# david8862/tf-keras-speech-commands

Hardware: AMD Instinct MI355X
Metric: 1 s@16 kHz clips/sec train-step, simple_cnn bs4096, 1/2/4/8 MI355X; eval top-1 (higher is better)
Workload: dtype f32; 1 GPU; configs[1]: simple_cnn train step = featurize(f32 1 s @16 kHz) + fwd + bwd + Adam, 36 logits (background + 35 words), batch 4096 per GPU; global_batch=4096, parallelism=dp1, gradient_exchange=none (one rank), rccl_ranks=0, library_build=bf45ad6cdf97

## Files before the change

### tf-keras-speech-commands_amd/csrc/kws_conv.h

```cpp
#pragma once
#include "kws_device.h"

namespace kws {

struct ConvGeom {
    int B, H, W, Ho, Wo;
    int stride, pt, pl;
    int KH, KW;
    int pmajor = 0;
};

enum { EPI_NONE = 0, EPI_RELU = 1, EPI_BIAS_RELU6 = 2, EPI_BIAS = 3, EPI_BIAS_RELU = 4,
       EPI_BN_RELU6 = 5,
       EPI_BNBWD_GATE6 = 6 };
enum { MODE_FWD = 0, MODE_DGRAD = 1 };

__host__ __device__ constexpr int stride16(int c) { return (c % 32 == 16) ? c : c + 16; }

template <int CR, int CO, int MODE, int EPI>
__global__ __launch_bounds__(256) void conv_gemm_kernel(const float *__restrict__ src, const float *__restrict__ wgt,
                                                         const float *__restrict__ bias, float *__restrict__ dst,
                                                         ConvGeom g)
{
    constexpr int KC = CR >= 32 ? 32 : CR;
// ... 1374 lines not shown
template <bool GBN = false>
__global__ __launch_bounds__(256, 2) void conv_wgrad_clip_bf16_kernel(const float *__restrict__ x, const float *__restrict__ dz,
                                                                       float *__restrict__ dw, int B, int H, int W, BnBwdArgs bn)
{
    constexpr int CIN = 16, COUT = 32, KS = 5;
    extern __shared__ __attribute__((aligned(16))) unsigned char ctile[];
    const int lane = threadIdx.x & 63, wave = __builtin_amdgcn_readfirstlane(threadIdx.x >> 6), li = lane & 15, lq = lane >> 4;
    const int nt = wave & 1, tg = wave >> 1;
    const int HP = H + 2, WP = W + 2, HW = H * W, NPIX = HP * WP;
    const int XPL = NPIX * 32, DPL = (HW + 1) * 32;
    unsigned char *Xs = ctile, *Ds = ctile + 3 * XPL;
    for (int i = threadIdx.x; i < (3 * XPL + 6 * DPL) / 4; i += 256) reinterpret_cast<unsigned *>(ctile)[i] = 0u;

    int xaddr[KS][2], daddr[KS][2];
#pragma unroll
    for (int ks = 0; ks < KS; ++ks)
#pragma unroll
        for (int rd = 0; rd < 2; ++rd) {
            const int pq = 32 * ks + 16 * rd + 4 * lq + (li >> 2);
            const bool ok = pq < HW;
            const int oh = ok ? pq / W : 0, ow = ok ? pq - oh * W : 0;
            xaddr[ks][rd] = (oh * WP + ow) * 32 + (li & 3) * 8;
            daddr[ks][rd] = (ok ? pq : HW) * 32 + (li & 3) * 8 + nt * DPL;
        }
    auto frag = [&](const unsigned char *p0, const unsigned char *p1) -> bf16x8 {
        union { struct { s16x4 lo, hi; } s; bf16x8 v; } u;
        u.s.lo = lds_read_tr16(p0);
        u.s.hi = lds_read_tr16(p1);
        return u.v;
    };

    f32x4 acc[5];
#pragma unroll
    for (int t = 0; t < 5; ++t) acc[t] = (f32x4){0.f, 0.f, 0.f, 0.f};

    constexpr int PX = 3, PD = 5;
    const int nx4 = HW * (CIN / 4), nd4 = HW * (COUT / 4);
    f32x4 px[PX], pd[PD], pz[GBN ? PD : 1];
    unsigned pa[GBN ? PD : 1];
    constexpr int F4 = COUT / 4;
    float gi[4], mean[4], inv[4], k2[4], k3[4];
    const int Wp = W / 2, nwin = (H / 2) * Wp;
    int cq[GBN ? PD : 1], ce[GBN ? PD : 1];
    if (GBN) {
#pragma unroll
        for (int e = 0; e < 4; ++e) {
            const int c = 4 * (threadIdx.x % F4) + e;
            inv[e] = bn.inv[c]; gi[e] = bn.gamma[c] * inv[e]; mean[e] = bn.mean[c];
            if (!bn.acc) { k2[e] = bn.k2[c]; k3[e] = bn.k3[c]; }
        }
        if (bn.acc) bn_bwd_k_from_acc(bn, COUT, threadIdx.x % F4, false, k2, k3);
#pragma unroll
        for (int j = 0; j < PD; ++j) {
            const int i = threadIdx.x + 256 * j, pix = i / F4, c4 = i % F4, y = pix / W, xx = pix - y * W;
            const bool in = i < nd4 && y < 2 * (H / 2) && xx < 2 * Wp;
            cq[j] = in ? ((y >> 1) * Wp + (xx >> 1)) * F4 + c4 : -1;
            ce[j] = (y & 1) * 2 + (xx & 1);
        }
    }
    auto prefetch = [&](int b) {
        const f32x4 *xs = reinterpret_cast<const f32x4 *>(x + (long)b * HW * CIN);
#pragma unroll
        for (int j = 0; j < PX; ++j) { const int i = threadIdx.x + 256 * j; px[j] = i < nx4 ? xs[i] : (f32x4){0.f, 0.f, 0.f, 0.f}; }
        if (GBN) {
            const f32x4 *zs = reinterpret_cast<const f32x4 *>(bn.z + (long)b * HW * COUT);
            const f32x4 *gws = reinterpret_cast<const f32x4 *>(bn.gw) + (long)b * nwin * F4;
            const unsigned *ars = reinterpret_cast<const unsigned *>(bn.arg) + (long)b * nwin * F4;
#pragma unroll
            for (int j = 0; j < PD; ++j) {
                const int i = threadIdx.x + 256 * j, q = cq[j] >= 0 ? cq[j] : 0;
                pd[j] = gws[q];
                pa[j] = ars[q];
                pz[j] = i < nd4 ? zs[i] : (f32x4){0.f, 0.f, 0.f, 0.f};
            }
        } else {
            const f32x4 *ds = reinterpret_cast<const f32x4 *>(dz + (long)b * HW * COUT);
#pragma unroll
            for (int j = 0; j < PD; ++j) { const int i = threadIdx.x + 256 * j; pd[j] = i < nd4 ? ds[i] : (f32x4){0.f, 0.f, 0.f, 0.f}; }
        }
    };
    auto form_dz = [&](int j) {
        f32x4 v = pd[j];
#pragma unroll
        for (int e = 0; e < 4; ++e) {
            const float g = (cq[j] >= 0 && (int)((pa[j] >> (8 * e)) & 0xFFu) == ce[j]) ? v[e] : 0.f;
            v[e] = gi[e] * (g - k2[e] - (pz[j][e] - mean[e]) * inv[e] * k3[e]);
        }
        return v;
    };
    auto stage_x = [&](int i, f32x4 v) {
        const int pix = i >> 2, c4 = i & 3, y = pix / W, xx = pix - y * W;
        bf16x4 h, m, l;
        split_bf16(v, h, m, l);
        unsigned char *d = Xs + ((y + 1) * WP + xx + 1) * 32 + c4 * 8;
        *reinterpret_cast<bf16x4 *>(d) = h;
        *reinterpret_cast<bf16x4 *>(d + XPL) = m;
        *reinterpret_cast<bf16x4 *>(d + 2 * XPL) = l;
    };
    auto stage_d = [&](int i, f32x4 v) {
        const int pix = i >> 3, c4 = i & 7;
        bf16x4 h, m, l;
        split_bf16(v, h, m, l);
        unsigned char *d = Ds + (c4 >> 2) * DPL + pix * 32 + (c4 & 3) * 8;
        *reinterpret_cast<bf16x4 *>(d) = h;
        *reinterpret_cast<bf16x4 *>(d + 2 * DPL) = m;
        *reinterpret_cast<bf16x4 *>(d + 4 * DPL) = l;
    };
    if ((int)blockIdx.x < B) prefetch(blockIdx.x);
    for (int b = blockIdx.x; b < B; b += gridDim.x) {
        __syncthreads();
#pragma unroll
        for (int j = 0; j < PX; ++j) { const int i = threadIdx.x + 256 * j; if (i < nx4) stage_x(i, px[j]); }
#pragma unroll
        for (int j = 0; j < PD; ++j) { const int i = threadIdx.x + 256 * j; if (i < nd4) stage_d(i, GBN ? form_dz(j) : pd[j]); }
        if (!GBN && (nx4 > 256 * PX || nd4 > 256 * PD)) {
            const f32x4 *xs = reinterpret_cast<const f32x4 *>(x + (long)b * HW * CIN);
            for (int i = threadIdx.x + 256 * PX; i < nx4; i += 256) stage_x(i, xs[i]);
            const f32x4 *ds = reinterpret_cast<const f32x4 *>(dz + (long)b * HW * COUT);
            for (int i = threadIdx.x + 256 * PD; i < nd4; i += 256) stage_d(i, ds[i]);
        }
        __syncthreads();
        if (b + (int)gridDim.x < B) prefetch(b + gridDim.x);
#pragma unroll
        for (int ks = 0; ks < KS; ++ks) {
            bf16x8 bfr[3];
#pragma unroll
            for (int p = 0; p < 3; ++p) bfr[p] = frag(Ds + 2 * p * DPL + daddr[ks][0], Ds + 2 * p * DPL + daddr[ks][1]);
#pragma unroll
            for (int t = 0; t < 5; ++t) {
                const int tap = tg + 2 * t;
                if (tap < 9) {
                    const int toff = ((tap / 3) * WP + tap % 3) * 32;
                    bf16x8 afr[3];
#pragma unroll
                    for (int p = 0; p < 3; ++p) afr[p] = frag(Xs + p * XPL + toff + xaddr[ks][0], Xs + p * XPL + toff + xaddr[ks][1]);
                    acc[t] = mfma_bf16x6(afr, bfr, acc[t]);
                }
            }
        }
    }
    __syncthreads();
    float *red = reinterpret_cast<float *>(ctile);
#pragma unroll
    for (int t = 0; t < 5; ++t) {
        const int tap = tg + 2 * t;
        if (tap < 9)
#pragma unroll
            for (int r = 0; r < 4; ++r) red[(tap * CIN + 4 * lq + r) * COUT + 16 * nt + li] = acc[t][r];
    }
    __syncthreads();
    for (int idx = threadIdx.x; idx < 9 * CIN * COUT; idx += 256) atomicAdd(dw + idx, red[idx]);
}

template <int COUT>
__global__ __launch_bounds__(256) void conv_wgrad_clip_kernel(const float *__restrict__ x, const float *__restrict__ dz,
                                                               float *__restrict__ dw, int B, int H, int W)
{
    constexpr int CIN = 16, NT = COUT / 16, XS = 16, DS = stride16(COUT);
    extern __shared__ __attribute__((aligned(16))) float smem[];
    const int lane = threadIdx.x & 63, wave = threadIdx.x >> 6, li = lane & 15, lq = lane >> 4;
    const int HP = H + 2, WP = W + 2, HW = H * W, nstep = (HW + 3) / 4;
    float *xt = smem;
    float *dt = smem + HP * WP * XS;
    for (int i = threadIdx.x; i < HP * WP * XS + 4 * nstep * DS; i += 256) smem[i] = 0.f;

    f32x4 acc[9][NT];
#pragma unroll
    for (int t = 0; t < 9; ++t)
#pragma unroll
        for (int nt = 0; nt < NT; ++nt) acc[t][nt] = (f32x4){0.f, 0.f, 0.f, 0.f};

    constexpr int PX = 3, PD = 5;
    const int nx4 = HW * (CIN / 4), nd4 = HW * (COUT / 4);
    float4 px[PX], pd[PD];
    auto prefetch = [&](int b) {
        const float4 *xs = reinterpret_cast<const float4 *>(x + (long)b * HW * CIN);
        const float4 *ds = reinterpret_cast<const float4 *>(dz + (long)b * HW * COUT);
#pragma unroll
        for (int j = 0; j < PX; ++j) { const int i = threadIdx.x + 256 * j; px[j] = i < nx4 ? xs[i] : make_float4(0.f, 0.f, 0.f, 0.f); }
#pragma unroll
        for (int j = 0; j < PD; ++j) { const int i = threadIdx.x + 256 * j; pd[j] = i < nd4 ? ds[i] : make_float4(0.f, 0.f, 0.f, 0.f); }
    };
    if ((int)blockIdx.x < B) prefetch(blockIdx.x);
    for (int b = blockIdx.x; b < B; b += gridDim.x) {
        __syncthreads();
#pragma unroll
        for (int j = 0; j < PX; ++j) {
            const int i = threadIdx.x + 256 * j;
            if (i < nx4) {
                const int pix = i / (CIN / 4), c4 = i % (CIN / 4), y = pix / W, xx = pix % W;
                *reinterpret_cast<float4 *>(&xt[((y + 1) * WP + xx + 1) * XS + 4 * c4]) = px[j];
            }
        }
#pragma unroll
        for (int j = 0; j < PD; ++j) {
            const int i = threadIdx.x + 256 * j;
            if (i < nd4) *reinterpret_cast<float4 *>(&dt[(i / (COUT / 4)) * DS + 4 * (i % (COUT / 4))]) = pd[j];
        }
        if (nx4 > 256 * PX || nd4 > 256 * PD) {
            const float4 *xs = reinterpret_cast<const float4 *>(x + (long)b * HW * CIN);
            for (int i = threadIdx.x + 256 * PX; i < nx4; i += 256) {
                const int pix = i / (CIN / 4), c4 = i % (CIN / 4), y = pix / W, xx = pix % W;
                *reinterpret_cast<float4 *>(&xt[((y + 1) * WP + xx + 1) * XS + 4 * c4]) = xs[i];
            }
            const float4 *ds = reinterpret_cast<const float4 *>(dz + (long)b * HW * COUT);
            for (int i = threadIdx.x + 256 * PD; i < nd4; i += 256)
                *reinterpret_cast<float4 *>(&dt[(i / (COUT / 4)) * DS + 4 * (i % (COUT / 4))]) = ds[i];
        }
        __syncthreads();
        if (b + (int)gridDim.x < B) prefetch(b + gridDim.x);
        for (int st = wave; st < nstep; st += 4) {
            const int p = 4 * st + lq, pc = p < HW ? p : HW - 1;
            const int oh = pc / W, ow = pc % W;
            float bf[NT];
#pragma unroll
            for (int nt = 0; nt < NT; ++nt) bf[nt] = dt[p * DS + 16 * nt + li];
            const float *a0 = &xt[(oh * WP + ow) * XS + li];
#pragma unroll
            for (int kh = 0; kh < 3; ++kh)
#pragma unroll
                for (int kw = 0; kw < 3; ++kw) {
                    const float a = a0[(kh * WP + kw) * XS];
#pragma unroll
                    for (int nt = 0; nt < NT; ++nt) acc[kh * 3 + kw][nt] = mfma16(a, bf[nt], acc[kh * 3 + kw][nt]);
                }
        }
    }
    float *red = smem;
#pragma unroll
    for (int t = 0; t < 9; ++t) {
#pragma unroll
        for (int nt = 0; nt < NT; ++nt) {
            __syncthreads();
            *reinterpret_cast<f32x4 *>(&red[(wave * 64 + lane) * 4]) = acc[t][nt];
            __syncthreads();
            if (wave == 0) {
                const f32x4 s0 = *reinterpret_cast<const f32x4 *>(&red[(0 * 64 + lane) * 4]);
                const f32x4 s1 = *reinterpret_cast<const f32x4 *>(&red[(1 * 64 + lane) * 4]);
                const f32x4 s2 = *reinterpret_cast<const f32x4 *>(&red[(2 * 64 + lane) * 4]);
                const f32x4 s3 = *reinterpret_cast<const f32x4 *>(&red[(3 * 64 + lane) * 4]);
#pragma unroll
                for (int r = 0; r < 4; ++r) red[1024 + (4 * lq + r) * COUT + 16 * nt + li] = (s0[r] + s1[r]) + (s2[r] + s3[r]);
            }
        }
        __syncthreads();
        for (int idx = threadIdx.x; idx < 16 * COUT; idx += 256) atomicAdd(dw + (long)t * CIN * COUT + idx, red[1024 + idx]);
    }
}

}
```

### tf-keras-speech-commands_amd/csrc/kws_model.hip

```cpp
#include <cstdlib>
#include <cstring>
#include <string>
#include <vector>

#include "kws_common.h"
#include "kws_model_types.h"
#include "kws_conv.h"
#include "kws_layers.h"
#include "kws_layer1.h"
#include "kws_layer1_moments.h"
#include "kws_layer1_fast.h"
#include "kws_lite.h"
#include "kws_lite_f16.h"
#include "kws_infer_fused.h"
#include "kws_conv_group.h"
#include "kws_dense_head.h"

using namespace kws;

namespace {

inline int same_out(int n, int s) { return (n + s - 1) / s; }
inline int same_pad_before(int n, int k, int s)
{
// ... 690 lines not shown
        } else if (fused_head) {
            const kws_train_args *a = fused_head;
            const HeadFwdArgs hf{params + m->o_hb, a->labels, a->class_weights, a->probs, w.loss_i, w.correct_i, a->grad_scale / (float)B, a->ignore_index};
            KWS_TRY(run_head_bwd(m, B, params, w.d1, nullptr, w.dd1, grads, true, s, grads + m->o_db, nullptr, nullptr, nullptr, false, &hf));
        } else
            KWS_TRY(run_head_bwd(m, B, params, w.d1, w.dlogits, w.dd1, grads, true, s, fuse && !det ? grads + m->o_db : nullptr, w.loss_i, w.correct_i,
                                 fuse ? stats : nullptr, det));
        fork0_bound = stop_event_bound(fork0_ev);
        if (fused_head) {
            if (fused_head->forward_event) KWS_HIP_CHECK(hipEventRecord(static_cast<hipEvent_t>(fused_head->forward_event), s));
            if (hook) KWS_TRY(hook->fire(1, s));
        }
    }
    {
        ConvGeom g;
        g.B = B; g.H = d.H4; g.W = d.W4; g.Ho = 1; g.Wo = 1; g.stride = 1; g.pt = 0; g.pl = 0; g.KH = d.H4; g.KW = d.W4;
        const bool hook_ev_here = hook && hook->wants(2) && hook->ev;
        if (hook) KWS_TRY(hook->fire(2, s, fork0_bound && hook_ev_here));
        if (hook_ev_here) {
            KWS_HIP_CHECK(hipStreamWaitEvent(s2, fork0_ev, 0));
        } else {
            if (!fork0_bound) KWS_HIP_CHECK(hipEventRecord(R->ev[0], s));
            KWS_HIP_CHECK(hipStreamWaitEvent(s2, R->ev[0], 0));
        }
        if (fused_head && stats) KWS_LAUNCH("loss_reduce_kernel", loss_reduce_kernel, dim3(1), dim3(256), 0, s2, w.loss_i, w.correct_i, B, stats);
        KWS_TRY(launch_wgrad<128, 128, 1>(w.a[3], w.dd1, grads + m->o_dk, g, s2, det));
        int nblk, rows;
        stat_grid(B, 128, nblk, rows);
        if (!head_bwd_fuses(m) || det) {
            KWS_LAUNCH("channel_stats_kernel.dense", channel_stats_kernel, dim3(nblk), dim3(256), 0, s, w.dd1, (long)B, 128, rows, w.partial);
            KWS_LAUNCH("colsum_finalize_kernel", colsum_finalize_kernel, dim3(128), dim3(256), 0, s, w.partial, nblk, 128, grads + m->o_db);
        }
        if (dense_fused) ;
        else if (mprec == 1) KWS_TRY_NB(launch_bf16<128, 128, MODE_DGRAD, EPI_NONE>("conv_bf16_dgrad", w.dd1, w.wsp[2], nullptr, w.da4, g, s));
        else KWS_TRY(launch_dgrad<128, 128, 1>(w.dd1, params + m->o_dk, w.da4, g, s));
        if (hook) KWS_TRY(hook->fire(3, s));
    }
    int fused_bn3_blocks = 0;
    for (int l = 3; l >= 1; --l) {
        if (hook && l == 2) KWS_TRY(hook->fire(5, s));
        const int C = kCh[l + 1];
        const long M = (long)B * Hz[l] * Wz[l];
        const float *da = l == 3 ? w.da4 : w.da[l];
        BnCoef k = coef_of(w.coef[l], C);
        int nblk, rows;
        stat_grid(M, C, nblk, rows);
        const float rate = (l == 3 && seed != 0) ? 0.5f : 0.f;
        const bool compact_g = l == 1 && cnn_compact_g2(m, mprec == 1);
        if (pool[l]) {
            const long NW = (long)B * (Hz[l] / 2) * (Wz[l] / 2);
            stat_grid(NW, C, nblk, rows);
            if (l == 1 && acc_bn2) ;
            else if (l == 3 && acc_bn4) ;
            else if (compact_g && routed_bwd2)
                KWS_LAUNCH(prof_name("bn_bwd_reduce_pool_kernel", l + 1), bn_bwd_reduce_routed_kernel, dim3(nblk), dim3(256), 0, s, w.zmax2, w.da[1], k, NW, C,
                           rows, w.partial);
            else if (compact_g)
                KWS_LAUNCH(prof_name("bn_bwd_reduce_pool_kernel", l + 1), bn_bwd_reduce_pool_kernel<true>, dim3(nblk), dim3(256), 0, s, w.z[l], w.da[1], k,
                           w.gz[l], B, Hz[l], Wz[l], C, rows, w.partial, rate, slo, shi, reinterpret_cast<unsigned char *>(w.da[2]));
            else if (l == 3 && mprec == 1)
                KWS_LAUNCH(prof_name("bn_bwd_reduce_pool_kernel", l + 1), bn_bwd_reduce_routed_full_kernel, dim3(nblk), dim3(256), 0, s, w.zmax4, w.arg4, da, k,
                           w.gz[l], B, Hz[l], Wz[l], C, rows, w.partial, rate, slo, shi);
            else
                KWS_LAUNCH(prof_name("bn_bwd_reduce_pool_kernel", l + 1), bn_bwd_reduce_pool_kernel<false>, dim3(nblk), dim3(256), 0, s, w.z[l],
                           const_cast<float *>(da), k, w.gz[l], B, Hz[l], Wz[l], C, rows, w.partial, rate, slo, shi);
        } else if (l == 2 && fused_bn3_blocks > 0)
            nblk = fused_bn3_blocks;
        else
            KWS_LAUNCH(prof_name("bn_bwd_reduce_kernel", l + 1), bn_bwd_reduce_kernel<false>, dim3(nblk), dim3(256), 0, s, w.z[l], da, k, w.gz[l], B, Hz[l], Wz[l], C,
                       rows, w.partial, rate, slo, shi);
        const bool wgrad_early_l1 = compact_g && Hs[1] * Ws[1] <= 160 && Hs[1] * Ws[1] * 8 <= 1280 && Hs[1] * Ws[1] * 4 <= 768;
        const bool acc_l = (l == 1 && acc_bn2) || (l == 2 && acc_bn3 && fused_bn3_blocks > 0) || (l == 3 && acc_bn4);
        const BnAccBwd ab{acc_set(R, 1, l, bpar[l]), acc_set(R, 1, l, bpar[l] + 1), M, grads + m->o_g[l], grads + m->o_b[l]};
        if (acc_l) ;
        else {
            if (l == 1 && wgrad_early_l1) arm(1);
            KWS_LAUNCH(prof_name("bn_bwd_finalize_kernel", l + 1), bn_bwd_finalize_kernel, dim3(C), dim3(64), 0, s, w.partial, nblk, M, C, params + m->o_g[l],
                       grads + m->o_g[l], grads + m->o_b[l], k);
        }
        if (l != 1) arm(l);
        if (l == 1)
            ;
        else if (l == 3 && acc_bn4)
            KWS_LAUNCH(prof_name("bn_bwd_apply_planes_kernel", l + 1), bn_bwd_apply_routed_planes_kernel<true>, dim3(std::min<unsigned>(1024u, blocks_for(M * C / 4, 256))),
                       dim3(256), 0, s, w.z[l], w.da4, w.arg4, k, params + m->o_g[l], B, Hz[l], Wz[l], C, ab, (Bf16PlanesOut{{w.dzp[0], w.dzp[1], w.dzp[2]}}));
        else if (l == 2 && acc_l)
            KWS_LAUNCH(prof_name("bn_bwd_apply_kernel", l + 1), bn_bwd_apply_acc_kernel<false>, dim3(std::min<unsigned>(1024u, blocks_for(M * C / 4, 256))), dim3(256), 0, s,
                       w.z[l], w.gz[l], k, params + m->o_g[l], M * C / 4, C, ab);
        else if (l == 3 && mprec == 1)
            KWS_LAUNCH(prof_name("bn_bwd_apply_planes_kernel", l + 1), bn_bwd_apply_planes_kernel<true>, dim3(blocks_for(M * C / 4, 256)), dim3(256), 0, s,
                       w.z[l], w.gz[l], k, params + m->o_g[l], M * C / 4, C, (Bf16PlanesOut{{w.dzp[0], w.dzp[1], w.dzp[2]}}));
        else if (l == 3)
            KWS_LAUNCH(prof_name("bn_bwd_apply_kernel", l + 1), bn_bwd_apply_kernel<true>, dim3(blocks_for(M * C, 256)), dim3(256), 0, s, w.z[l], w.gz[l], k,
                       params + m->o_g[l], M * C, C);
        else
            KWS_LAUNCH(prof_name("bn_bwd_apply_kernel", l + 1), bn_bwd_apply_kernel<false>, dim3(blocks_for(M * C, 256)), dim3(256), 0, s, w.z[l], w.gz[l], k,
                       params + m->o_g[l], M * C, C);
        const float *in = w.a[l - 1];
        float *dk = grads + m->o_k[l];
        const float *kern = params + m->o_k[l];
        if (hook && l == 3) KWS_TRY(hook->fire(4, s));
        if (l != 1)
            if (int rc = fork(l)) return rc;
        if (l == 3) {
            const ConvGeom g = geom3x3(B, Hs[3], Ws[3], 1);
            if (mprec == 1 && cnn_a3_on_load(m, true, true))
                KWS_TRY((launch_wgrad_bf16<64, 128, 1, true, true>(w.z[2], nullptr, dk, g, s2, w.dzp, det, coef_of(w.coef[2], 64).scale)));
            else if (mprec == 1) KWS_TRY(launch_wgrad_bf16<64, 128, 1, true>(in, nullptr, dk, g, s2, w.dzp, det));
            else KWS_TRY(launch_wgrad<64, 128, 1>(in, w.gz[3], dk, g, s2, det));
            if (comm) KWS_TRY(comm_allreduce_early(comm, grads + m->o_k[3], m->P - m->o_k[3], s2));
            if (bucket_event) KWS_HIP_CHECK(hipEventRecord(bucket_event, s2));
            if (group_bwd) {
                fused_bn3_blocks = launch_group_dgrad4(m, B, w, s, acc_bn3 ? acc_set(R, 1, 2, bpar[2]) : nullptr);
                if (fused_bn3_blocks < 0) return fused_bn3_blocks;
            } else if (mprec == 1 && blocks_for((long)B * Hs[3] * Ws[3], 64) <= (unsigned)kStatStride) {
                const BnCoef k3 = coef_of(w.coef[2], 64);
                fused_bn3_blocks = launch_bf16<128, 64, MODE_DGRAD, EPI_BNBWD_GATE6>("conv_bf16_dgrad", nullptr, w.wsp[1], k3.scale, w.gz[2], g, s, w.partial,
                                                                                   w.z[2], w.dzp);
                if (fused_bn3_blocks < 0) return fused_bn3_blocks;
            } else if (mprec == 1)
                KWS_TRY_NB(launch_bf16<128, 64, MODE_DGRAD, EPI_NONE>("conv_bf16_dgrad", nullptr, w.wsp[1], nullptr, w.da[2], g, s, nullptr, nullptr, w.dzp));
            else KWS_TRY(launch_dgrad<128, 64, 1>(w.gz[3], kern, w.da[2], g, s));
        } else if (l == 2) {
            const ConvGeom g = geom3x3(B, Hs[2], Ws[2], 2);
            if (mprec == 1) KWS_TRY(launch_wgrad_bf16<32, 64, 3>(in, w.gz[2], dk, g, s2, nullptr, det));
            else KWS_TRY(launch_wgrad<32, 64, 3>(in, w.gz[2], dk, g, s2, det));
            if (group_bwd) {
                if (acc_bn2) arm(1);
                KWS_TRY(launch_group_dgrad3(m, B, w, s, acc_bn2 ? acc_set(R, 1, 1, bpar[1]) : nullptr));
            }
            else KWS_TRY(launch_dgrad<64, 32, 2>(w.gz[2], kern, w.da[1], g, s));
        } else {
            const int H1 = Hs[1], W1 = Ws[1];
            auto even_grid = [&](int max_blocks) { const int cpb = (B + max_blocks - 1) / max_blocks; return (unsigned)((B + cpb - 1) / cpb); };
            const unsigned nblk = even_grid(cu_count() * 3), nblk_d = even_grid(cu_count() * 5);
            const size_t smw = sizeof(float) * ((size_t)(H1 + 2) * (W1 + 2) * 16 + (size_t)((H1 * W1 + 3) / 4) * 4 * stride16(32));
            const size_t smw2 = std::max(smw, sizeof(float) * (size_t)(1024 + 16 * 32));
            const size_t smd = sizeof(float) * (size_t)(H1 + 2) * (W1 + 2) * (32 + 4);
            BnBwdArgs bn = {w.z[1], params + m->o_g[1], k.mean, k.inv, k.k2, k.k3};
            if (compact_g) { bn.gw = w.da[1]; bn.arg = routed_bwd2 ? w.arg2 : reinterpret_cast<const unsigned char *>(w.da[2]); }
            BnBwdArgs bn_w = bn;
            if (acc_bn2) {
                bn.acc = bn_w.acc = acc_set(R, 1, 1, bpar[1]);
                bn.M = bn_w.M = M;
                bn.acc_clear_set = acc_set(R, 1, 1, bpar[1] + 1);
                bn.dgamma = grads + m->o_g[1]; bn.dbeta = grads + m->o_b[1]; bn.k2w = k.k2; bn.k3w = k.k3;
            }
            const bool wgrad_bf16 = mprec == 1 && H1 * W1 <= 160;
            const bool wgrad_early = compact_g && wgrad_bf16 && H1 * W1 * 8 <= 1280 && H1 * W1 * 4 <= 768;
            const size_t smwb = std::max((size_t)3 * 32 * (H1 + 2) * (W1 + 2) + (size_t)6 * 32 * (H1 * W1 + 1), sizeof(float) * 9 * 16 * 32);
            auto wgrad_grid = [&](int occ) { return dim3(det ? 1u : even_grid(cu_count() * std::min(occ, 2))); };
            if (wgrad_early) {
                if (int rc = fork(1)) return rc;
                static const int occ = resident_blocks(conv_wgrad_clip_bf16_kernel<true>, 256, smwb);
                if (!no_arm) arm_stop_event(R->ev[9], s2);
                KWS_LAUNCH("conv_wgrad_clip_bf16<16,32>", conv_wgrad_clip_bf16_kernel<true>, wgrad_grid(occ), dim3(256), smwb, s2, in, nullptr, dk, B, H1, W1, bn_w);
            }
            if (mprec == 1) {
                const size_t smdb = (size_t)12 * 16 * (((H1 + 2) * (W1 + 2) + 15) & ~15);
                if (wgrad_early)
                    KWS_LAUNCH("conv_dgrad_clip_bf16<32,16>", (conv_dgrad_clip_bf16_kernel<true, true, false>), dim3(even_grid(cu_count() * 2)), dim3(256), smdb, s,
                               w.gz[1], kern, w.da[0], B, H1, W1, bn);
                else if (compact_g)
                    KWS_LAUNCH("conv_dgrad_clip_bf16<32,16>", (conv_dgrad_clip_bf16_kernel<true, true>), dim3(even_grid(cu_count() * 2)), dim3(256), smdb, s,
                               w.gz[1], kern, w.da[0], B, H1, W1, bn);
                else
                    KWS_LAUNCH("conv_dgrad_clip_bf16<32,16>", (conv_dgrad_clip_bf16_kernel<true, false>), dim3(even_grid(cu_count() * 2)), dim3(256), smdb, s,
                               w.gz[1], kern, w.da[0], B, H1, W1, bn);
            } else
                KWS_LAUNCH("conv_dgrad_clip<32,16>", (conv_dgrad_clip_kernel<32, true>), dim3(nblk_d), dim3(256), smd, s, w.gz[1], kern, w.da[0], B, H1, W1, bn);
            if (wgrad_early) {
                ;
            } else if (wgrad_bf16) {
                if (int rc = fork(1)) return rc;
                static const int occ = resident_blocks(conv_wgrad_clip_bf16_kernel<false>, 256, smwb);
                KWS_LAUNCH("conv_wgrad_clip_bf16<16,32>", conv_wgrad_clip_bf16_kernel<false>, wgrad_grid(occ), dim3(256), smwb, s2, in, w.gz[1], dk, B, H1, W1, bn);
            } else {
                if (int rc = fork(1)) return rc;
                KWS_LAUNCH("conv_wgrad_clip<16,32>", conv_wgrad_clip_kernel<32>, dim3(det ? 1u : nblk), dim3(256), smw2, s2, in, w.gz[1], dk, B, H1, W1);
            }
        }
    }
    {
        const int cpb = std::max(1, (B + kMaxStatBlocks - 1) / kMaxStatBlocks), nb = (B + cpb - 1) / cpb;
        const size_t smem1 = sizeof(float) * (size_t)(d.H0 + 2) * (d.W0 + 2);
        const bool l1m = d.H0 % 2 == 0 && d.W0 % 2 == 0 && (d.H0 + 2) * (d.W0 + 2) <= 64 * kL1Stage &&
                         (d.H0 / 2) * (d.W0 / 2) <= 4 * kL1MaxTiles;
        const int cpw = std::max(1, (B + 4 * kMaxStatBlocks - 1) / (4 * kMaxStatBlocks)), nbm = (B + 4 * cpw - 1) / (4 * cpw);
        const size_t smemm = sizeof(float) * 4 * (d.H0 == 30 && d.W0 == 20 ? (size_t)L1Runs<30, 20>::TILE : (size_t)((((d.H0 + 2) * (d.W0 + 2)) + 3) & ~3));
        const long M1 = (long)B * d.H0 * d.W0;
        BnCoef k1 = coef_of(w.coef[0], 16);
        const float *kern1 = params + m->o_k[0];
        if (l1m) {
            const double *q = moments ? moments : w.moments;
            const bool fin_in_kernel = acc_ok && d.H0 == 30 && d.W0 == 20;
            if (fin_in_kernel) {
                double *acc0 = acc_set(R, 1, 0, 0);
                const L1FinalizeArgs fin{acc0, reinterpret_cast<unsigned *>(acc0 + kAccDoubles - 1), q, params + m->o_g[0], grads + m->o_k[0],
                                         grads + m->o_g[0], grads + m->o_b[0]};
                KWS_LAUNCH("l1m_bwd_onepass_kernel", (l1f_bwd_onepass_kernel<30, 20>), dim3(nbm), dim3(256), smemm, s, feat, kern1, w.da[0], k1, B, cpw, w.partial, fin);
            } else if (d.H0 == 30 && d.W0 == 20)
                KWS_LAUNCH("l1m_bwd_onepass_kernel", (l1f_bwd_onepass_kernel<30, 20>), dim3(nbm), dim3(256), smemm, s, feat, kern1, w.da[0], k1, B, cpw, w.partial);
            else
                KWS_LAUNCH("l1m_bwd_onepass_kernel", l1m_bwd_onepass_kernel, dim3(nbm), dim3(256), smemm, s, feat, kern1, w.da[0], k1, B, d.H0, d.W0, cpw,
                           w.partial);
            if (!fin_in_kernel)
                KWS_LAUNCH("l1_bwd_finalize_moments_kernel", l1_bwd_finalize_moments_kernel, dim3(144 + 16), dim3(64), 0, s, w.partial, nbm, q, kern1,
                           params + m->o_g[0], k1, grads + m->o_k[0], grads + m->o_g[0], grads + m->o_b[0]);
        } else {
            KWS_LAUNCH("l1_bwd_reduce_kernel", l1_bwd_reduce_kernel<16>, dim3(nb), dim3(256), smem1, s, feat, kern1, w.da[0], k1, B, d.H0, d.W0,
                       cpb, w.partial);
            KWS_LAUNCH(prof_name("bn_bwd_finalize_kernel", 1), bn_bwd_finalize_kernel, dim3(16), dim3(64), 0, s, w.partial, nb, M1, 16,
                       params + m->o_g[0], grads + m->o_g[0], grads + m->o_b[0], k1);
            KWS_LAUNCH("l1_bwd_wgrad_kernel", l1_bwd_wgrad_kernel<16>, dim3(det ? 1 : nb), dim3(256), smem1, s, feat, kern1, w.da[0], k1, params + m->o_g[0],
                       grads + m->o_k[0], B, d.H0, d.W0, det ? B : cpb);
        }
    }
    if (!stop_event_bound(R->ev[9])) KWS_HIP_CHECK(hipEventRecord(R->ev[9], s2));
    KWS_HIP_CHECK(hipStreamWaitEvent(s, R->ev[9], 0));
    KWS_LAUNCH_CHECK("simple_cnn backward");
    R->acc_dirty = false;
    return KWS_OK;
}


ConvGeom geom1x1(int B, int H, int W)
{
    ConvGeom g;
    g.B = B; g.H = H; g.W = W; g.Ho = H; g.Wo = W; g.stride = 1; g.pt = 0; g.pl = 0; g.KH = 1; g.KW = 1;
    return g;
}


static int lite_forward_f16(const kws_model *m, const float *feat, int B, const float *params, const float *state, CnnWs &w, float *probs,
                            int32_t *argmax, hipStream_t s)
{
    const CnnDims &d = m->d;
    const bool front_ok = d.H0 % 2 == 0 && d.W0 % 2 == 0 && (d.H0 + 2) * (d.W0 + 2) <= 64 * 12 && d.H2 >= 1 && d.W2 >= 1;
    if (!front_ok || d.H2 * d.W2 > kF16MaxN2 || d.H3 * d.W3 > kF16MaxP3 || d.H4 < 1 || d.W4 < 1 || m->C > kF16HeadCols || d.flat > kWdRow)
        return fail(KWS_ERR_UNSUPPORTED, "fp16 inference of simple_cnn_lite needs a feature map up to about 30 x 20 and at most %d classes "
                                         "(got %d x %d, %d classes): use KWS_INFER_FP32", kF16HeadCols, d.H0, d.W0, m->C);
    const bool prepared = m->prepared_for(params, state, w.base, B, matrix_prec(m), infer_prec(m));
    _Float16 *blob = reinterpret_cast<_Float16 *>(w.partial);
    if (!prepared) {
        if (int rc = infer_coefs(m, params, state, w, s)) return rc;
        KWS_LAUNCH("lite_f16_prepare_kernel", lite_f16_prepare_kernel, dim3(32), dim3(256), 0, s, params + m->o_pwk[2], params + m->o_pwk[3],
                   params + m->o_dk, params + m->o_hk, m->C, d.flat, blob);
    }
    BnCoef k0 = coef_of(w.coef[0], 16), k1 = coef_of(w.coef[1], 32), k2 = coef_of(w.coef[2], 64), k3 = coef_of(w.coef[3], 128);
    const LiteFrontArgs fa = {params + m->o_dwk[0], params + m->o_pwk[0], params + m->o_pwb[0], k0.scale, k0.shift,
                              params + m->o_dwk[1], params + m->o_pwk[1], params + m->o_pwb[1], k1.scale, k1.shift};
    const size_t sm = sizeof(float) * (size_t)lite_front_floats(d.H0, d.W0);
    const int waves = cu_count() * std::max(1, std::min(8, (int)(160 * 1024 / sm)));
    const int cpw = std::max(1, (B + waves - 1) / waves), nblk = (B + cpw - 1) / cpw;
    _Float16 *a2h = reinterpret_cast<_Float16 *>(w.a[1]);
    KWS_LAUNCH("lite_front_infer_kernel", lite_front_infer_kernel, dim3(nblk), dim3(64), sm, s, feat, fa, w.a[1], B, d.H0, d.W0, cpw, a2h);
    LiteF16Args a;
    a.dwk3 = params + m->o_dwk[2]; a.pwb3 = params + m->o_pwb[2]; a.sc3 = k2.scale; a.sh3 = k2.shift;
    a.dwk4 = params + m->o_dwk[3]; a.pwb4 = params + m->o_pwb[3]; a.sc4 = k3.scale; a.sh4 = k3.shift;
    a.db = params + m->o_db; a.hb = params + m->o_hb; a.blob = blob;
    a.C = m->C; a.H2 = d.H2; a.W2 = d.W2; a.H3 = d.H3; a.W3 = d.W3;
    a.pt3 = same_pad_before(d.H2, 3, 2); a.pl3 = same_pad_before(d.W2, 3, 2); a.H4 = d.H4; a.W4 = d.W4;
    if (int rc = ensure_dynamic_lds(reinterpret_cast<const void *>(lite_back_f16_kernel), kF16LdsBytes)) return rc;
    const int ntile = (B + kF16Clips - 1) / kF16Clips;
    KWS_LAUNCH("lite_back_f16_kernel", lite_back_f16_kernel, dim3(std::min(ntile, cu_count())), dim3(256), (size_t)kF16LdsBytes, s, a2h, a, B, probs, argmax);
    KWS_LAUNCH_CHECK("simple_cnn_lite fp16 forward");
    return KWS_OK;
}

int lite_forward(const kws_model *m, const float *feat, int B, const float *params, float *state, CnnWs &w, bool training,
                 uint64_t seed, hipStream_t s)
{
    const CnnDims &d = m->d;
    const int Hs[4] = {d.H0, d.H1, d.H2, d.H3}, Ws[4] = {d.W0, d.W1, d.W2, d.W3};
    const int Hz[4] = {d.H0, d.H1, d.H3, d.H3}, Wz[4] = {d.W0, d.W1, d.W3, d.W3};
    const int strd[4] = {1, 1, 2, 1};
    const bool pool[4] = {true, true, false, true};
    const uint32_t slo = (uint32_t)(seed & 0xFFFFFFFFu), shi = (uint32_t)(seed >> 32);
    int l_begin = 0;
    if (!training && !m->prepared_for(params, state, w.base, B, matrix_prec(m), infer_prec(m)))
        if (int rc = infer_coefs(m, params, state, w, s)) return rc;
    if (!training && d.H0 % 2 == 0 && d.W0 % 2 == 0 && (d.H0 + 2) * (d.W0 + 2) <= 64 * 12 && d.H2 >= 1 && d.W2 >= 1) {
        BnCoef k0 = coef_of(w.coef[0], 16), k1 = coef_of(w.coef[1], 32);
        const LiteFrontArgs fa = {params + m->o_dwk[0], params + m->o_pwk[0], params + m->o_pwb[0], k0.scale, k0.shift,
                                  params + m->o_dwk[1], params + m->o_pwk[1], params + m->o_pwb[1], k1.scale, k1.shift};
        const size_t sm = sizeof(float) * (size_t)lite_front_floats(d.H0, d.W0);
        const int waves = cu_count() * std::max(1, std::min(8, (int)(160 * 1024 / sm)));
        const int cpw = std::max(1, (B + waves - 1) / waves), nblk = (B + cpw - 1) / cpw;
        KWS_LAUNCH("lite_front_infer_kernel", lite_front_infer_kernel, dim3(nblk), dim3(64), sm, s, feat, fa, w.a[1], B, d.H0, d.W0, cpw);
        l_begin = 2;
    }
    for (int l = l_begin; l < 4; ++l) {
        const float *in = l == 0 ? feat : w.a[l - 1];
        const int Cin = kCh[l], C = kCh[l + 1];
        const long M = (long)B * Hz[l] * Wz[l];
        const ConvGeom g = geom3x3(B, Hs[l], Ws[l], strd[l]);
        KWS_LAUNCH(prof_name("dwconv_fwd_kernel", l + 1), dwconv_fwd_kernel, dim3(blocks_for(M * Cin, 256)), dim3(256), 0, s, in,
                   params + m->o_dwk[l], w.dwo[l], g, Cin);
        const float *pwk = params + m->o_pwk[l], *pwb = params + m->o_pwb[l];
        const ConvGeom g1 = geom1x1(B, Hz[l], Wz[l]);
        if (l == 0) KWS_LAUNCH("pw1_fwd_kernel", pw1_fwd_kernel<16>, dim3(blocks_for(M * 16, 256)), dim3(256), 0, s, w.dwo[0], pwk, pwb, w.z[0], M);
        else if (l == 1) KWS_TRY(launch_gemm<16, 32, MODE_FWD, EPI_BIAS>(w.dwo[1], pwk, pwb, w.z[1], g1, s));
        else if (l == 2) KWS_TRY(launch_gemm<32, 64, MODE_FWD, EPI_BIAS_RELU>(w.dwo[2], pwk, pwb, w.z[2], g1, s));
        else KWS_TRY(launch_gemm<64, 128, MODE_FWD, EPI_BIAS_RELU>(w.dwo[3], pwk, pwb, w.z[3], g1, s));
        BnCoef k = coef_of(w.coef[l], C);
        if (training) {
            int nblk, rows;
            stat_grid(M, C, nblk, rows);
            KWS_LAUNCH(prof_name("channel_stats_kernel", l + 1), channel_stats_kernel, dim3(nblk), dim3(256), 0, s, w.z[l], M, C, rows, w.partial);
// ... 560 lines not shown
```

Measured before the change: 7.560 million clips/s.

## Add software-pipelined double-buffered wgrad kernel specialized for 15x10 layer-1 shape

Adds a 512-thread weight-gradient kernel for the second conv layer, specialized at compile time for a 15x10 feature map. It double-buffers LDS tiles and prefetches the next clip's inputs into registers while the MFMAs run on the current one. Work is split across waves by tap, with the centre tap shared and reduced at the end. The aim is to hide global-load and bf16-split staging latency behind the matrix ops and to cut per-iteration sync. In exchange it uses a larger LDS footprint and one block per CU, and it only runs for that exact shape in non-deterministic mode.

After: 7.660 million clips/s (median of 6 runs). +1.3%, better.

```diff
diff --git a/tf-keras-speech-commands_amd/csrc/kws_conv.h b/tf-keras-speech-commands_amd/csrc/kws_conv.h
--- a/tf-keras-speech-commands_amd/csrc/kws_conv.h
+++ b/tf-keras-speech-commands_amd/csrc/kws_conv.h
@@ -1550,6 +1550,165 @@
     for (int idx = threadIdx.x; idx < 9 * CIN * COUT; idx += 256) atomicAdd(dw + idx, red[idx]);
 }
 
+template <int H, int W>
+__global__ __launch_bounds__(512, 4) void conv_wgrad_clip_bf16_pipe_kernel(const float *__restrict__ x, float *__restrict__ dw, int B,
+                                                                            BnBwdArgs bn)
+{
+    constexpr int CIN = 16, COUT = 32, NTH = 512, F4 = COUT / 4;
+    constexpr int HW = H * W, KS = (HW + 31) / 32;
+    constexpr int XP = W + 8, XROWS = (32 * KS - 1) / W + 3 > H + 2 ? (32 * KS - 1) / W + 3 : H + 2;
+    constexpr int XPL = XROWS * XP * 32, DPL = 32 * KS * 32;
+    constexpr int BUF = 3 * XPL + 6 * DPL;
+    constexpr int NX4 = HW * (CIN / 4), ND4 = HW * (COUT / 4), PX = (NX4 + NTH - 1) / NTH, PD = (ND4 + NTH - 1) / NTH;
+    constexpr int Wp = W / 2, NWIN = (H / 2) * Wp;
+    static_assert(W + 2 <= XP && (XP - W) % 8 == 0, "x slot pitch");
+    static_assert(NTH % F4 == 0, "a thread's dz channels are the same in every unit");
+    static_assert(12 * CIN * COUT * 4 <= 2 * BUF, "the partial tiles fit the staging space");
+    extern __shared__ __attribute__((aligned(16))) unsigned char ctile[];
+    const int tid = threadIdx.x, lane = tid & 63, wave = __builtin_amdgcn_readfirstlane(tid >> 6), li = lane & 15, lq = lane >> 4;
+    const int nt = wave >> 2, qq = (wave + nt) & 3;
+    int toff2[2];
+#pragma unroll
+    for (int t = 0; t < 2; ++t) toff2[t] = (((2 * qq + t) / 3) * XP + (2 * qq + t) % 3) * 32;
+    typedef unsigned u32x4 __attribute__((ext_vector_type(4)));
+    for (int i = tid; i < 2 * BUF / 16; i += NTH) reinterpret_cast<u32x4 *>(ctile)[i] = (u32x4){0u, 0u, 0u, 0u};
+
+    int xaddr[KS][2];
+#pragma unroll
+    for (int ks = 0; ks < KS; ++ks)
+#pragma unroll
+        for (int rd = 0; rd < 2; ++rd) {
+            const int pq = 32 * ks + 16 * rd + 4 * lq + (li >> 2);
+            xaddr[ks][rd] = ((pq / W) * XP + pq % W) * 32 + (li & 3) * 8;
+        }
+    const int daddr = (4 * lq + (li >> 2)) * 32 + (li & 3) * 8 + nt * DPL;
+    auto frag = [&](const unsigned char *p0, const unsigned char *p1) -> bf16x8 {
+        union { struct { s16x4 lo, hi; } s; bf16x8 v; } u;
+        u.s.lo = lds_read_tr16(p0);
+        u.s.hi = lds_read_tr16(p1);
+        return u.v;
+    };
+
+    f32x4 acc[3];
+#pragma unroll
+    for (int t = 0; t < 3; ++t) acc[t] = (f32x4){0.f, 0.f, 0.f, 0.f};
+
+    float gi[4], mean[4], inv[4], k2[4], k3[4];
+#pragma unroll
+    for (int e = 0; e < 4; ++e) {
+        const int c = 4 * (tid % F4) + e;
+        inv[e] = bn.inv[c]; gi[e] = bn.gamma[c] * inv[e]; mean[e] = bn.mean[c];
+        if (!bn.acc) { k2[e] = bn.k2[c]; k3[e] = bn.k3[c]; }
+    }
+    if (bn.acc) bn_bwd_k_from_acc(bn, COUT, tid % F4, false, k2, k3);
+    int cw[PD];
+#pragma unroll
+    for (int j = 0; j < PD; ++j) {
+        const int i = tid + NTH * j, pix = i / F4, c4 = i % F4, y = pix / W, xx = pix % W;
+        const bool in = i < ND4 && y < 2 * (H / 2) && xx < 2 * Wp;
+        cw[j] = in ? ((((y >> 1) * Wp + (xx >> 1)) * F4 + c4) << 2) | ((y & 1) * 2 + (xx & 1)) : -1;
+    }
+
+    f32x4 px[PX], pd[PD], pz[PD];
+    unsigned pa[PD];
+    auto prefetch = [&](int b) {
+        const f32x4 *xs = reinterpret_cast<const f32x4 *>(x + (long)b * HW * CIN);
+        const f32x4 *zs = reinterpret_cast<const f32x4 *>(bn.z + (long)b * HW * COUT);
+        const f32x4 *gws = reinterpret_cast<const f32x4 *>(bn.gw) + (long)b * NWIN * F4;
+        const unsigned *ars = reinterpret_cast<const unsigned *>(bn.arg) + (long)b * NWIN * F4;
+#pragma unroll
+        for (int j = 0; j < PX; ++j) {
+            const int i = tid + NTH * j;
+            if (NTH * (j + 1) <= NX4 || i < NX4) px[j] = xs[i];
+        }
+#pragma unroll
+        for (int j = 0; j < PD; ++j) {
+            const int i = tid + NTH * j, q = cw[j] >= 0 ? cw[j] >> 2 : 0;
+            if (NTH * (j + 1) <= ND4 || i < ND4) { pd[j] = gws[q]; pa[j] = ars[q]; pz[j] = zs[i]; }
+        }
+    };
+    auto stage = [&](unsigned char *buf) {
+#pragma unroll
+        for (int j = 0; j < PX; ++j) {
+            const int i = tid + NTH * j, pix = i >> 2, c4 = i & 3;
+            if (NTH * (j + 1) <= NX4 || i < NX4) {
+                bf16x4 h, m, l;
+                split_bf16(px[j], h, m, l);
+                unsigned char *d = buf + ((pix / W + 1) * XP + pix % W + 1) * 32 + c4 * 8;
+                *reinterpret_cast<bf16x4 *>(d) = h;
+                *reinterpret_cast<bf16x4 *>(d + XPL) = m;
+                *reinterpret_cast<bf16x4 *>(d + 2 * XPL) = l;
+            }
+        }
+#pragma unroll
+        for (int j = 0; j < PD; ++j) {
+            const int i = tid + NTH * j, pix = i >> 3, c4 = i & 7;
+            if (NTH * (j + 1) <= ND4 || i < ND4) {
+                f32x4 v = pd[j];
+#pragma unroll
+                for (int e = 0; e < 4; ++e) {
+                    const float g = (cw[j] >= 0 && (int)((pa[j] >> (8 * e)) & 0xFFu) == (cw[j] & 3)) ? v[e] : 0.f;
+                    v[e] = gi[e] * (g - k2[e] - (pz[j][e] - mean[e]) * inv[e] * k3[e]);
+                }
+                bf16x4 h, m, l;
+                split_bf16(v, h, m, l);
+                unsigned char *d = buf + 3 * XPL + (c4 >> 2) * DPL + pix * 32 + (c4 & 3) * 8;
+                *reinterpret_cast<bf16x4 *>(d) = h;
+                *reinterpret_cast<bf16x4 *>(d + 2 * DPL) = m;
+                *reinterpret_cast<bf16x4 *>(d + 4 * DPL) = l;
+            }
+        }
+    };
+    auto mma = [&](const unsigned char *buf) {
+        const unsigned char *Xs = buf, *Ds = buf + 3 * XPL;
+#pragma unroll
+        for (int ks = 0; ks < KS; ++ks) {
+            bf16x8 bfr[3];
+#pragma unroll
+            for (int p = 0; p < 3; ++p) bfr[p] = frag(Ds + 2 * p * DPL + daddr + ks * 1024, Ds + 2 * p * DPL + daddr + ks * 1024 + 512);
+#pragma unroll
+            for (int t = 0; t < 3; ++t) {
+                if (t == 2 && ks % 4 != qq) continue;
+                const int toff = t < 2 ? toff2[t] : (2 * XP + 2) * 32;
+                bf16x8 afr[3];
+#pragma unroll
+                for (int p = 0; p < 3; ++p) afr[p] = frag(Xs + p * XPL + toff + xaddr[ks][0], Xs + p * XPL + toff + xaddr[ks][1]);
+                acc[t] = mfma_bf16x6(afr, bfr, acc[t]);
+            }
+        }
+    };
+
+    const int G = gridDim.x;
+    int b = blockIdx.x;
+    if (b < B) prefetch(b);
+    __syncthreads();
+    if (b < B) stage(ctile);
+    if (b + G < B) prefetch(b + G);
+    __syncthreads();
+    for (int it = 0; b < B; b += G, ++it) {
+        unsigned char *cur = ctile + (it & 1) * BUF, *nxt = ctile + ((it & 1) ^ 1) * BUF;
+        if (b + G < B) stage(nxt);
+        if (b + 2 * G < B) prefetch(b + 2 * G);
+        mma(cur);
+        __syncthreads();
+    }
+    float *red = reinterpret_cast<float *>(ctile);
+    constexpr int T1 = CIN * COUT;
+#pragma unroll
+    for (int t = 0; t < 3; ++t)
+#pragma unroll
+        for (int r = 0; r < 4; ++r) red[((t < 2 ? 2 * qq + t : 8 + qq) * CIN + 4 * lq + r) * COUT + 16 * nt + li] = acc[t][r];
+    __syncthreads();
+    for (int idx = tid; idx < 9 * T1; idx += NTH)
+        atomicAdd(dw + idx, idx < 8 * T1 ? red[idx] : red[idx] + red[idx + T1] + red[idx + 2 * T1] + red[idx + 3 * T1]);
+}
+template <int H, int W>
+constexpr size_t wgrad_clip_pipe_lds()
+{
+    constexpr int KS = (H * W + 31) / 32, XP = W + 8, XROWS = (32 * KS - 1) / W + 3 > H + 2 ? (32 * KS - 1) / W + 3 : H + 2;
+    return (size_t)2 * (3 * XROWS * XP * 32 + 6 * 32 * KS * 32);
+}
+
 template <int COUT>
 __global__ __launch_bounds__(256) void conv_wgrad_clip_kernel(const float *__restrict__ x, const float *__restrict__ dz,
                                                                float *__restrict__ dw, int B, int H, int W)
diff --git a/tf-keras-speech-commands_amd/csrc/kws_model.hip b/tf-keras-speech-commands_amd/csrc/kws_model.hip
--- a/tf-keras-speech-commands_amd/csrc/kws_model.hip
+++ b/tf-keras-speech-commands_amd/csrc/kws_model.hip
@@ -866,9 +866,16 @@
             auto wgrad_grid = [&](int occ) { return dim3(det ? 1u : even_grid(cu_count() * std::min(occ, 2))); };
             if (wgrad_early) {
                 if (int rc = fork(1)) return rc;
-                static const int occ = resident_blocks(conv_wgrad_clip_bf16_kernel<true>, 256, smwb);
                 if (!no_arm) arm_stop_event(R->ev[9], s2);
-                KWS_LAUNCH("conv_wgrad_clip_bf16<16,32>", conv_wgrad_clip_bf16_kernel<true>, wgrad_grid(occ), dim3(256), smwb, s2, in, nullptr, dk, B, H1, W1, bn_w);
+                if (!det && H1 == 15 && W1 == 10) {
+                    constexpr size_t smp = wgrad_clip_pipe_lds<15, 10>();
+                    if (int rc = ensure_dynamic_lds(reinterpret_cast<const void *>(conv_wgrad_clip_bf16_pipe_kernel<15, 10>), (int)smp)) return rc;
+                    KWS_LAUNCH("conv_wgrad_clip_bf16<16,32>", (conv_wgrad_clip_bf16_pipe_kernel<15, 10>), dim3(even_grid(cu_count())), dim3(512), smp, s2, in, dk, B,
+                               bn_w);
+                } else {
+                    static const int occ = resident_blocks(conv_wgrad_clip_bf16_kernel<true>, 256, smwb);
+                    KWS_LAUNCH("conv_wgrad_clip_bf16<16,32>", conv_wgrad_clip_bf16_kernel<true>, wgrad_grid(occ), dim3(256), smwb, s2, in, nullptr, dk, B, H1, W1, bn_w);
+                }
             }
             if (mprec == 1) {
                 const size_t smdb = (size_t)12 * 16 * (((H1 + 2) * (W1 + 2) + 15) & ~15);
```
